# PengjieRen/CaSE_RG

Hardware: AMD Instinct MI355X
Metric: train tokens/sec (query+passage) CaSE model (higher is better)
Workload: dtype bf16; 1 GPU; CaSE train step fwd+bwd+allreduce+clip+Adam+EMA, d_model=512, 6 encoder layers, 10 passages x 384 tok, query 64, answer 40, vocab 30522, per-GPU batch 32, dropout on; global_batch=32, parallelism=dp1

## Files before the change

case_rg_amd/csrc/elementwise.hip:

```cpp
#include "common.h"

namespace {

constexpr int EW_THREADS = 256;

template <typename T>
__global__ void add_kernel(const T* __restrict__ a, const T* __restrict__ b, T* __restrict__ o, int64_t n) {
  for (int64_t i = (int64_t)blockIdx.x * blockDim.x + threadIdx.x; i < n; i += (int64_t)gridDim.x * blockDim.x)
    Elem<T>::st(o + i, Elem<T>::ld(a + i) + Elem<T>::ld(b + i));
}

template <typename T>
__global__ void dropout_kernel(const T* __restrict__ x, T* __restrict__ y, int64_t n, float p, uint64_t seed,
                               uint64_t offset, const CaseStepState* state) {
  offset += rng_base_of(state);
  const float scale = 1.f / (1.f - p);
  for (int64_t i = (int64_t)blockIdx.x * blockDim.x + threadIdx.x; i < n; i += (int64_t)gridDim.x * blockDim.x)
    Elem<T>::st(y + i, rng_uniform(seed, offset + (uint64_t)i) >= p ? Elem<T>::ld(x + i) * scale : 0.f);
}

template <typename T>
__global__ void mask_rows_kernel(const T* __restrict__ x, const uint8_t* __restrict__ valid, T* __restrict__ y,
                                 int64_t rows, int64_t cols) {
  const int64_t n = rows * cols;
// ... 52 lines not shown
      for (int r = 0; r < 8; ++r) t += part[r][c];
      atomicAdd(out + gc, t);
    }
  }
}

template <typename T>
__global__ void add_vec_kernel(const T* __restrict__ a, const T* __restrict__ b, T* __restrict__ o, int64_t nvec) {
  constexpr int E = Vec16<T>::N;
  for (int64_t i = (int64_t)blockIdx.x * blockDim.x + threadIdx.x; i < nvec; i += (int64_t)gridDim.x * blockDim.x) {
    float x[E], y[E];
    Vec16<T>::load(a + i * E, x);
    Vec16<T>::load(b + i * E, y);
#pragma unroll
    for (int e = 0; e < E; ++e) x[e] += y[e];
    Vec16<T>::store(o + i * E, x);
  }
}

struct AddNArgs {
  const void* src[8];
  int n;
};
template <typename T>
__global__ void add_n_vec_kernel(const AddNArgs a, T* __restrict__ o, int64_t nvec) {
  constexpr int E = Vec16<T>::N;
  for (int64_t i = (int64_t)blockIdx.x * blockDim.x + threadIdx.x; i < nvec; i += (int64_t)gridDim.x * blockDim.x) {
    float acc[E], y[E];
    Vec16<T>::load(reinterpret_cast<const T*>(a.src[0]) + i * E, acc);
#pragma unroll
    for (int j = 1; j < 8; ++j) {
      if (j < a.n) {
        Vec16<T>::load(reinterpret_cast<const T*>(a.src[j]) + i * E, y);
#pragma unroll
        for (int e = 0; e < E; ++e) acc[e] += y[e];
      }
    }
    Vec16<T>::store(o + i * E, acc);
  }
}

template <typename T>
__global__ void dropout_vec_kernel(const T* __restrict__ x, T* __restrict__ y, int64_t nvec, float p, uint64_t seed,
                                   uint64_t offset, const CaseStepState* state) {
  offset += rng_base_of(state);
  constexpr int E = Vec16<T>::N;
  const float scale = 1.f / (1.f - p);
  for (int64_t i = (int64_t)blockIdx.x * blockDim.x + threadIdx.x; i < nvec; i += (int64_t)gridDim.x * blockDim.x) {
    float v[E];
    Vec16<T>::load(x + i * E, v);
    const uint64_t idx0 = offset + (uint64_t)(i * E);
    if ((idx0 & 1) == 0) {
#pragma unroll
      for (int e = 0; e < E; e += 2) {
        float u0, u1;
        rng_uniform2(seed, idx0 + e, u0, u1);
        v[e] = u0 >= p ? v[e] * scale : 0.f;
        v[e + 1] = u1 >= p ? v[e + 1] * scale : 0.f;
      }
    } else {
#pragma unroll
      for (int e = 0; e < E; ++e) v[e] = rng_uniform(seed, idx0 + e) >= p ? v[e] * scale : 0.f;
    }
    Vec16<T>::store(y + i * E, v);
  }
}

template <typename T>
__global__ void mask_rows_vec_kernel(const T* __restrict__ x, const uint8_t* __restrict__ valid, T* __restrict__ y,
                                     int64_t rows, int64_t cols) {
  constexpr int E = Vec16<T>::N;
  const int64_t vpr = cols / E, nvec = rows * vpr;
  const bool in_place = x == y;
  for (int64_t i = (int64_t)blockIdx.x * blockDim.x + threadIdx.x; i < nvec; i += (int64_t)gridDim.x * blockDim.x) {
    const bool ok = valid[i / vpr] != 0;
    if (in_place && ok) continue;
    float v[E];
    if (ok) Vec16<T>::load(x + i * E, v);
    else {
#pragma unroll
      for (int e = 0; e < E; ++e) v[e] = 0.f;
    }
    Vec16<T>::store(y + i * E, v);
  }
}

template <typename T>
__global__ __launch_bounds__(256) void rowdot_fwd_kernel(const T* __restrict__ x, const float* __restrict__ w,
                                                         const float* __restrict__ b, float* __restrict__ y, int64_t rows,
                                                         int64_t cols) {
  const int lane = threadIdx.x & 63;
  const int64_t wave = (int64_t)blockIdx.x * 4 + (threadIdx.x >> 6), nwaves = (int64_t)gridDim.x * 4;
  for (int64_t r = wave; r < rows; r += nwaves) {
    float acc = 0.f;
    for (int64_t c = lane; c < cols; c += 64) acc += Elem<T>::ld(x + r * cols + c) * w[c];
    acc = wave_sum(acc);
    if (lane == 0) y[r] = acc + (b ? b[0] : 0.f);
  }
}

struct SkinnyArgs {
  const void* x[4];
  int64_t width[4];
  const float* w; const float* b; float* y;
  int64_t rows, cols;
  int nseg, nout;
};
template <typename T, bool VEC>
__global__ __launch_bounds__(256) void linear_skinny_kernel(const SkinnyArgs a) {
  const int lane = threadIdx.x & 63;
  const int64_t wave = (int64_t)blockIdx.x * 4 + (threadIdx.x >> 6), nwaves = (int64_t)gridDim.x * 4;
  constexpr int NV = Vec16<T>::N;
  for (int64_t r = wave; r < a.rows; r += nwaves) {
    float acc[8] = {0.f, 0.f, 0.f, 0.f, 0.f, 0.f, 0.f, 0.f};
    int64_t off = 0;
#pragma unroll
    for (int k = 0; k < 4; ++k) {
      if (k < a.nseg) {
        const T* xr = reinterpret_cast<const T*>(a.x[k]) + r * a.width[k];
        if constexpr (VEC) {
#pragma unroll 2
          for (int64_t c = (int64_t)lane * NV; c < a.width[k]; c += 64 * NV) {
            float xv[NV];
            Vec16<T>::load(xr + c, xv);
#pragma unroll
            for (int o = 0; o < 8; ++o) {
              if (o < a.nout) {
                const float* wr = a.w + o * a.cols + off + c;
#pragma unroll
                for (int q = 0; q < NV / 4; ++q) {
                  const float4 wv = *reinterpret_cast<const float4*>(wr + 4 * q);
                  acc[o] = fmaf(xv[4 * q], wv.x, acc[o]);
                  acc[o] = fmaf(xv[4 * q + 1], wv.y, acc[o]);
                  acc[o] = fmaf(xv[4 * q + 2], wv.z, acc[o]);
                  acc[o] = fmaf(xv[4 * q + 3], wv.w, acc[o]);
                }
              }
            }
          }
        } else {
          for (int64_t c = lane; c < a.width[k]; c += 64) {
            const float xv = Elem<T>::ld(xr + c);
#pragma unroll
            for (int o = 0; o < 8; ++o)
              if (o < a.nout) acc[o] = fmaf(xv, a.w[o * a.cols + off + c], acc[o]);
          }
        }
        off += a.width[k];
      }
    }
#pragma unroll
    for (int o = 0; o < 8; ++o) {
      if (o < a.nout) {
        const float t = wave_sum(acc[o]);
        if (lane == 0) a.y[r * a.nout + o] = t + (a.b ? a.b[o] : 0.f);
      }
    }
  }
}

template <typename T>
__global__ __launch_bounds__(256) void rowdot_bwd_kernel(const float* __restrict__ g, const T* __restrict__ x,
                                                         const float* __restrict__ w, T* __restrict__ dx,
                                                         float* __restrict__ dw, float* __restrict__ db, int64_t rows,
                                                         int64_t cols, int row_splits) {
  __shared__ float part[4][64];
// ... 343 lines not shown
    }
    Vec16<T>::store(de + r * H + c, ge);
    Vec16<T>::store(da1 + r * H + c, g1);
    Vec16<T>::store(da2 + r * H + c, g2);
  }
}

template <typename T>
__global__ void max_over_p_fwd_kernel(const T* __restrict__ x, T* __restrict__ out, int32_t* __restrict__ arg, int64_t B,
                                      int64_t P, int64_t inner) {
  const int64_t n = B * inner;
  for (int64_t i = (int64_t)blockIdx.x * blockDim.x + threadIdx.x; i < n; i += (int64_t)gridDim.x * blockDim.x) {
    const int64_t b = i / inner, k = i % inner;
    float best = Elem<T>::ld(x + (b * P) * inner + k);
    int32_t bi = 0;
    for (int64_t p = 1; p < P; ++p) {
      const float v = Elem<T>::ld(x + (b * P + p) * inner + k);
      if (v > best) {
        best = v;
        bi = (int32_t)p;
      }
    }
    Elem<T>::st(out + i, best);
    arg[i] = bi;
  }
}

template <typename T>
__global__ void max_over_p_bwd_kernel(const T* __restrict__ d_out, const int32_t* __restrict__ arg, T* __restrict__ dx,
                                      int64_t B, int64_t P, int64_t inner) {
  const int64_t n = B * P * inner;
  for (int64_t i = (int64_t)blockIdx.x * blockDim.x + threadIdx.x; i < n; i += (int64_t)gridDim.x * blockDim.x) {
    const int64_t k = i % inner, bp = i / inner, b = bp / P, p = bp % P;
    Elem<T>::st(dx + i, arg[b * inner + k] == (int32_t)p ? Elem<T>::ld(d_out + b * inner + k) : 0.f);
  }
}

}

#define EW_DISPATCH(what, n_elems, KERNEL, ...)                                                              \
  do {                                                                                                       \
    const int grid = grid_for((n_elems), EW_THREADS, 4);                                                     \
    hipStream_t s_ = (hipStream_t)stream;                                                                    \
    if (dtype == CASE_F32) { typedef float T; hipLaunchKernelGGL(KERNEL<T>, dim3(grid), dim3(EW_THREADS), 0, s_, __VA_ARGS__); } \
    else if (dtype == CASE_BF16) { typedef bf16_t T; hipLaunchKernelGGL(KERNEL<T>, dim3(grid), dim3(EW_THREADS), 0, s_, __VA_ARGS__); } \
    else return case_set_error(CASE_E_UNSUPPORTED, what ": dtype %d", dtype);                              \
    return case_check_launch(what);                                                                          \
  } while (0)

extern "C" int case_add(const void* a, const void* b, void* out, int64_t n, int32_t dtype, case_stream_t stream) {
  CASE_REQUIRE(a && b && out && n > 0, "case_add: bad argument");
  const int ev = dtype == CASE_BF16 ? 8 : 4;
  if (n % ev == 0 && al16(a) && al16(b) && al16(out))
    EW_DISPATCH("case_add", n / ev, add_vec_kernel, (const T*)a, (const T*)b, (T*)out, n / ev);
  EW_DISPATCH("case_add", n, add_kernel, (const T*)a, (const T*)b, (T*)out, n);
}

extern "C" int case_add_n(const void* const* srcs, int32_t count, void* out, int64_t n, int32_t dtype, case_stream_t stream) {
  CASE_REQUIRE(srcs && out && n > 0 && count >= 2 && count <= 8, "case_add_n: bad argument (2 <= count <= 8)");
  const int ev = dtype == CASE_BF16 ? 8 : 4;
  CASE_REQUIRE(n % ev == 0 && al16(out), "case_add_n: element count must be a multiple of %d and the tensors 16-byte aligned", ev);
  AddNArgs a = {};
  a.n = count;
  for (int j = 0; j < count; ++j) {
    CASE_REQUIRE(srcs[j] && al16(srcs[j]), "case_add_n: null or misaligned source %d", j);
    a.src[j] = srcs[j];
  }
  EW_DISPATCH("case_add_n", n / ev, add_n_vec_kernel, a, (T*)out, n / ev);
}

extern "C" int case_dropout(const void* x, void* y, int64_t n, float p, uint64_t seed, uint64_t offset, const CaseStepState* state,
                            int32_t dtype, case_stream_t stream) {
  CASE_REQUIRE(x && y && n > 0 && p >= 0.f && p < 1.f, "case_dropout: bad argument");
  const int ev = dtype == CASE_BF16 ? 8 : 4;
  if (n % ev == 0 && al16(x) && al16(y))
    EW_DISPATCH("case_dropout", n / ev, dropout_vec_kernel, (const T*)x, (T*)y, n / ev, p, seed, offset, state);
  EW_DISPATCH("case_dropout", n, dropout_kernel, (const T*)x, (T*)y, n, p, seed, offset, state);
}

extern "C" int case_mask_rows(const void* x, const uint8_t* row_valid, void* y, int64_t rows, int64_t cols,
                              int32_t dtype, case_stream_t stream) {
  CASE_REQUIRE(x && row_valid && y && rows > 0 && cols > 0, "case_mask_rows: bad argument");
  const int ev = dtype == CASE_BF16 ? 8 : 4;
  if (cols % ev == 0 && al16(x) && al16(y))
    EW_DISPATCH("case_mask_rows", rows * cols / ev, mask_rows_vec_kernel, (const T*)x, row_valid, (T*)y, rows, cols);
  EW_DISPATCH("case_mask_rows", rows * cols, mask_rows_kernel, (const T*)x, row_valid, (T*)y, rows, cols);
}

static int colsum_splits(int64_t rows, int64_t cols) {
  const int64_t col_blocks = (cols + 63) / 64;
  int64_t want = 2048 / col_blocks;
  const int64_t cap = (rows + 31) / 32;
  if (want > cap) want = cap;
  return (int)(want < 1 ? 1 : want);
}

extern "C" int case_colsum(const void* x, float* out, int64_t rows, int64_t cols, int32_t dtype, case_stream_t stream) {
  CASE_REQUIRE(x && out && rows > 0 && cols > 0, "case_colsum: bad argument");
  {
    const int ev = dtype == CASE_BF16 ? 8 : 4;
    if (cols % ev == 0 && al16(x)) {
      const int64_t col_blocks = (cols + 32 * ev - 1) / (32 * ev);
      int64_t want = 2048 / col_blocks, cap = (rows + 63) / 64;
      if (want > cap) want = cap;
      if (want < 1) want = 1;
      const int vsplits = (int)want;
      hipStream_t vs = (hipStream_t)stream;
      if (dtype == CASE_F32) hipLaunchKernelGGL(colsum_vec_kernel<float>, dim3((unsigned)(col_blocks * vsplits)), dim3(256), 0, vs, (const float*)x, out, rows, cols, vsplits);
      else hipLaunchKernelGGL(colsum_vec_kernel<bf16_t>, dim3((unsigned)(col_blocks * vsplits)), dim3(256), 0, vs, (const bf16_t*)x, out, rows, cols, vsplits);
      return case_check_launch("case_colsum");
    }
  }
  const int splits = colsum_splits(rows, cols);
  const int grid = (int)((cols + 63) / 64) * splits;
  hipStream_t s = (hipStream_t)stream;
  if (dtype == CASE_F32) hipLaunchKernelGGL(colsum_kernel<float>, dim3(grid), dim3(256), 0, s, (const float*)x, out, rows, cols, splits);
  else hipLaunchKernelGGL(colsum_kernel<bf16_t>, dim3(grid), dim3(256), 0, s, (const bf16_t*)x, out, rows, cols, splits);
  return case_check_launch("case_colsum");
}

extern "C" int case_cast(const void* x, void* y, int64_t n, int32_t src, int32_t dst, case_stream_t stream) {
  CASE_REQUIRE(x && y && n > 0, "case_cast: bad argument");
  const int grid = grid_for(n, EW_THREADS, 4);
  hipStream_t s = (hipStream_t)stream;
  if (src == CASE_F32 && dst == CASE_BF16) hipLaunchKernelGGL((cast_kernel<float, bf16_t>), dim3(grid), dim3(EW_THREADS), 0, s, (const float*)x, (bf16_t*)y, n);
  else if (src == CASE_BF16 && dst == CASE_F32) hipLaunchKernelGGL((cast_kernel<bf16_t, float>), dim3(grid), dim3(EW_THREADS), 0, s, (const bf16_t*)x, (float*)y, n);
  else if (src == CASE_F32 && dst == CASE_F32) hipLaunchKernelGGL((cast_kernel<float, float>), dim3(grid), dim3(EW_THREADS), 0, s, (const float*)x, (float*)y, n);
  else if (src == CASE_BF16 && dst == CASE_BF16) hipLaunchKernelGGL((cast_kernel<bf16_t, bf16_t>), dim3(grid), dim3(EW_THREADS), 0, s, (const bf16_t*)x, (bf16_t*)y, n);
  else return case_set_error(CASE_E_UNSUPPORTED, "case_cast: dtype");
  return case_check_launch("case_cast");
}

extern "C" int case_scale_cols(const void* x, const float* w, void* y, int64_t rows, int64_t cols, int32_t dtype,
                               case_stream_t stream) {
  CASE_REQUIRE(x && w && y && rows > 0 && cols > 0, "case_scale_cols: bad argument");
  EW_DISPATCH("case_scale_cols", rows * cols, scale_cols_kernel, (const T*)x, w, (T*)y, rows, cols);
}

extern "C" int case_scale_cols_bwd(const void* dy, const void* x, const float* w, void* dx, float* dw, int64_t rows,
                                   int64_t cols, int32_t dtype, case_stream_t stream) {
  CASE_REQUIRE(dy && x && w && dx && dw && rows > 0 && cols > 0, "case_scale_cols_bwd: bad argument");
  const int splits = colsum_splits(rows, cols);
  const int grid = (int)((cols + 63) / 64) * splits;
  hipStream_t s = (hipStream_t)stream;
  if (dtype == CASE_F32) hipLaunchKernelGGL(scale_cols_bwd_kernel<float>, dim3(grid), dim3(256), 0, s, (const float*)dy, (const float*)x, w, (float*)dx, dw, rows, cols, splits);
  else hipLaunchKernelGGL(scale_cols_bwd_kernel<bf16_t>, dim3(grid), dim3(256), 0, s, (const bf16_t*)dy, (const bf16_t*)x, w, (bf16_t*)dx, dw, rows, cols, splits);
  return case_check_launch("case_scale_cols_bwd");
}

extern "C" int case_scale_add_rows(const void* x, const float* pe, void* y, int64_t rows, int64_t seq_len, int64_t H,
                                   float scale, int32_t dtype, case_stream_t stream) {
  CASE_REQUIRE(x && y && rows > 0 && seq_len > 0 && H > 0, "case_scale_add_rows: bad argument");
  EW_DISPATCH("case_scale_add_rows", rows * H, scale_add_rows_kernel, (const T*)x, pe, (T*)y, rows, seq_len, H, scale);
}

extern "C" int case_embed_pos_fwd(const int64_t* ids, const float* table, const float* pe, void* out, int64_t rows,
                                  int64_t seq_len, int64_t H, int64_t vocab, float scale, float drop_p, uint64_t seed,
                                  uint64_t offset, const CaseStepState* state, int32_t dtype, case_stream_t stream) {
  CASE_REQUIRE(ids && table && pe && out && rows > 0 && seq_len > 0 && H > 0 && vocab > 0, "case_embed_pos_fwd: bad argument");
  if ((dtype == CASE_BF16 || dtype == CASE_F32) && H % 8 == 0 && al16(table) && al16(pe) && al16(out) && rows * (H / 8) < (1ll << 31) &&
      seq_len < (1ll << 31)) {
    const unsigned chunks = (unsigned)(rows * (H / 8));
    const dim3 grid((unsigned)grid_for(chunks, 256, 1, 256 * 16));
    hipStream_t s_ = (hipStream_t)stream;
    if (dtype == CASE_F32)
      hipLaunchKernelGGL(embed_pos_fwd_vec_kernel<float>, grid, dim3(256), 0, s_, ids, table, pe, (float*)out, chunks, (unsigned)seq_len,
// ... 146 lines not shown
```

case_rg_amd/csrc/rowops.hip:

```cpp
#include <stdlib.h>

#ifndef CASE_STREAM_DEFAULT_POLICY
#define CASE_VEC16_NT
#endif
#include "common.h"

namespace {

constexpr int LN_THREADS = 256;
constexpr int LN_MAXPT = 16;

template <typename T>
__global__ __launch_bounds__(LN_THREADS) void ln_fwd_kernel(const T* __restrict__ x, const T* __restrict__ x2,
                                                            const float* __restrict__ gamma,
                                                            const float* __restrict__ beta, T* __restrict__ y,
                                                            float* __restrict__ mean, float* __restrict__ rstd,
                                                            int64_t rows, int64_t cols, float eps) {
  __shared__ float red[32];
  for (int64_t r = blockIdx.x; r < rows; r += gridDim.x) {
    const T* xr = x + r * cols;
    const T* x2r = x2 ? x2 + r * cols : nullptr;
    float s = 0.f;
    for (int64_t c = threadIdx.x; c < cols; c += LN_THREADS) s += Elem<T>::ld(xr + c) + (x2r ? Elem<T>::ld(x2r + c) : 0.f);
    const float mu = block_sum(s, red) / (float)cols;
// ... 48 lines not shown
    const float m1 = block_sum(s1, red) / (float)cols;
    const float m2 = block_sum(s2, red) / (float)cols;
    T* dxr = dx + r * cols;
#pragma unroll
    for (int i = 0; i < LN_MAXPT; ++i) {
      const int64_t c = threadIdx.x + (int64_t)i * LN_THREADS;
      if (c < cols) {
        const float xh = (Elem<T>::ld(xr + c) + (x2r ? Elem<T>::ld(x2r + c) : 0.f) - mu) * rs;
        const float g = Elem<T>::ld(dyr + c) * gamma[c];
        Elem<T>::st(dxr + c, rs * (g - m1 - xh * m2) + (dx_add ? Elem<T>::ld(dx_add + r * cols + c) : 0.f));
      }
    }
  }
#pragma unroll
  for (int i = 0; i < LN_MAXPT; ++i) {
    const int64_t c = threadIdx.x + (int64_t)i * LN_THREADS;
    if (c < cols) {
      atomicAdd(d_gamma + c, acc_g[i]);
      atomicAdd(d_beta + c, acc_b[i]);
    }
  }
}

constexpr int LNV_MAX = 8;

template <typename T, int NV>
__global__ __launch_bounds__(256) void ln_fwd_vec_kernel(const T* __restrict__ x, const T* __restrict__ x2,
                                                         const float* __restrict__ gamma, const float* __restrict__ beta,
                                                         T* __restrict__ y, float* __restrict__ mean,
                                                         float* __restrict__ rstd, int64_t rows, int64_t cols, float eps) {
  constexpr int E = Vec16<T>::N;
  const int lane = threadIdx.x & 63;
  const int64_t wave = (int64_t)blockIdx.x * 4 + (threadIdx.x >> 6), nwaves = (int64_t)gridDim.x * 4;
  for (int64_t r = wave; r < rows; r += nwaves) {
    float v[NV][E];
    float s = 0.f;
#pragma unroll
    for (int i = 0; i < NV; ++i) {
      const int64_t c = ((int64_t)i * 64 + lane) * E;
      if (c < cols) {
        Vec16<T>::load(x + r * cols + c, v[i]);
        if (x2) {
          float w[E];
          Vec16<T>::load(x2 + r * cols + c, w);
#pragma unroll
          for (int e = 0; e < E; ++e) v[i][e] += w[e];
        }
#pragma unroll
        for (int e = 0; e < E; ++e) s += v[i][e];
      }
    }
    const float mu = wave_sum(s) / (float)cols;
    float q = 0.f;
#pragma unroll
    for (int i = 0; i < NV; ++i)
      if (((int64_t)i * 64 + lane) * E < cols) {
#pragma unroll
        for (int e = 0; e < E; ++e) q += (v[i][e] - mu) * (v[i][e] - mu);
      }
    const float rs = rsqrtf(wave_sum(q) / (float)cols + eps);
    if (lane == 0) {
      mean[r] = mu;
      rstd[r] = rs;
    }
#pragma unroll
    for (int i = 0; i < NV; ++i) {
      const int64_t c = ((int64_t)i * 64 + lane) * E;
      if (c < cols) {
        float g[E], b[E], o[E];
#pragma unroll
        for (int e = 0; e < E; e += 4) {
          const float4 gg = *reinterpret_cast<const float4*>(gamma + c + e), bb = *reinterpret_cast<const float4*>(beta + c + e);
          g[e] = gg.x; g[e + 1] = gg.y; g[e + 2] = gg.z; g[e + 3] = gg.w;
          b[e] = bb.x; b[e + 1] = bb.y; b[e + 2] = bb.z; b[e + 3] = bb.w;
        }
#pragma unroll
        for (int e = 0; e < E; ++e) o[e] = (v[i][e] - mu) * rs * g[e] + b[e];
        Vec16<T>::store(y + r * cols + c, o);
      }
    }
  }
}

template <typename T, int NV>
__global__ __launch_bounds__(256) void ln_bwd_vec_guarded_kernel(const T* __restrict__ dy, const T* __restrict__ x,
                                                         const T* __restrict__ x2, const float* __restrict__ gamma,
                                                         const float* __restrict__ mean, const float* __restrict__ rstd,
                                                         T* __restrict__ dx, const T* __restrict__ dx_add,
                                                         float* __restrict__ d_gamma, float* __restrict__ d_beta, int64_t rows,
                                                         int64_t cols) {
  constexpr int E = Vec16<T>::N;
  extern __shared__ float part[];
  const int lane = threadIdx.x & 63, wid = threadIdx.x >> 6;
  const int64_t wave = (int64_t)blockIdx.x * 4 + wid, nwaves = (int64_t)gridDim.x * 4;
  float ag[NV][E], ab[NV][E], g[NV][E];
#pragma unroll
  for (int i = 0; i < NV; ++i) {
    const int64_t c = ((int64_t)i * 64 + lane) * E;
#pragma unroll
    for (int e = 0; e < E; ++e) {
      ag[i][e] = ab[i][e] = 0.f;
      g[i][e] = c < cols ? gamma[c + e] : 0.f;
    }
  }
  for (int64_t r = wave; r < rows; r += nwaves) {
    const float mu = mean[r], rs = rstd[r];
    float xh[NV][E], gy[NV][E];
    float s1 = 0.f, s2 = 0.f;
#pragma unroll
    for (int i = 0; i < NV; ++i) {
      const int64_t c = ((int64_t)i * 64 + lane) * E;
      if (c < cols) {
        float d[E];
        Vec16<T>::load(x + r * cols + c, xh[i]);
        if (x2) {
          float w[E];
          Vec16<T>::load(x2 + r * cols + c, w);
#pragma unroll
          for (int e = 0; e < E; ++e) xh[i][e] += w[e];
        }
        Vec16<T>::load(dy + r * cols + c, d);
#pragma unroll
        for (int e = 0; e < E; ++e) {
          xh[i][e] = (xh[i][e] - mu) * rs;
          gy[i][e] = d[e] * g[i][e];
          s1 += gy[i][e];
          s2 += gy[i][e] * xh[i][e];
          ag[i][e] += d[e] * xh[i][e];
          ab[i][e] += d[e];
        }
      }
    }
    const float m1 = wave_sum(s1) / (float)cols, m2 = wave_sum(s2) / (float)cols;
#pragma unroll
    for (int i = 0; i < NV; ++i) {
      const int64_t c = ((int64_t)i * 64 + lane) * E;
      if (c < cols) {
        float o[E];
#pragma unroll
        for (int e = 0; e < E; ++e) o[e] = rs * (gy[i][e] - m1 - xh[i][e] * m2);
        if (dx_add) {
          float w[E];
          Vec16<T>::load(dx_add + r * cols + c, w);
#pragma unroll
          for (int e = 0; e < E; ++e) o[e] += w[e];
        }
        Vec16<T>::store(dx + r * cols + c, o);
      }
    }
  }
  for (int w = 1; w < 4; ++w) {
    if (wid == w) {
#pragma unroll
      for (int i = 0; i < NV; ++i) {
        const int64_t c = ((int64_t)i * 64 + lane) * E;
        if (c < cols) {
#pragma unroll
          for (int e = 0; e < E; ++e) {
            part[c + e] = ag[i][e];
            part[cols + c + e] = ab[i][e];
          }
        }
      }
    }
    __syncthreads();
    if (wid == 0) {
// ... 30 lines not shown
  void* out;
  float p;
  uint64_t seed, offset;
  const CaseStepState* state;
};
template <typename T, typename V = Vec16<T>>
__device__ __forceinline__ void ln_store_dropped(const LnDrop& dr, int64_t idx, const float (&o)[V::N]) {
  constexpr int E = V::N;
  float q[E];
  if constexpr (sizeof(T) == 2) {
#pragma unroll
    for (int i = 0; i < E; i += 2) {
      const uint32_t w = f32x2_to_bf16x2(o[i], o[i + 1]);
      q[i] = __uint_as_float(w << 16);
      q[i + 1] = __uint_as_float(w & 0xffff0000u);
    }
  } else {
#pragma unroll
    for (int e = 0; e < E; ++e) q[e] = o[e];
  }
  const float scale = 1.f / (1.f - dr.p);
#pragma unroll
  for (int e = 0; e < E; e += 2) {
    float u0, u1;
    rng_uniform2(dr.seed, dr.offset + rng_base_of(dr.state) + (uint64_t)(idx + e), u0, u1);
    q[e] = u0 >= dr.p ? q[e] * scale : 0.f;
    q[e + 1] = u1 >= dr.p ? q[e + 1] * scale : 0.f;
  }
  V::store(reinterpret_cast<T*>(dr.out) + idx, q);
}

template <typename T, int NV, bool HAS_X2, bool HAS_ADD, bool DROP2 = false, typename V = Vec16<T>>
__global__ __launch_bounds__(256) void ln_bwd_vec_kernel(const T* __restrict__ dy, const T* __restrict__ x,
                                                         const T* __restrict__ x2, const float* __restrict__ gamma,
                                                         const float* __restrict__ mean, const float* __restrict__ rstd,
                                                         T* __restrict__ dx, const T* __restrict__ dx_add,
                                                         float* __restrict__ d_gamma, float* __restrict__ d_beta, int64_t rows,
                                                         int64_t cols, const LnDrop dr = LnDrop()) {
  constexpr int E = V::N;
  typedef typename V::raw raw_t;
  extern __shared__ float part[];
  const int lane = threadIdx.x & 63, wid = threadIdx.x >> 6;
  const int64_t wave = (int64_t)blockIdx.x * 4 + wid, nwaves = (int64_t)gridDim.x * 4;
  float ag[NV][E], ab[NV][E], g[NV][E];
#pragma unroll
  for (int i = 0; i < NV; ++i) {
    const int64_t c = ((int64_t)i * 64 + lane) * E;
#pragma unroll
    for (int e = 0; e < E; ++e) {
      ag[i][e] = ab[i][e] = 0.f;
      g[i][e] = gamma[c + e];
    }
  }
  struct Raw {
    raw_t x[NV], d[NV], x2[HAS_X2 ? NV : 1], add[HAS_ADD ? NV : 1];
    float mu, rs;
  };
  auto request = [&](Raw& w, int64_t r) {
    const int64_t base = r * cols + (int64_t)lane * E;
    w.mu = mean[r];
    w.rs = rstd[r];
#pragma unroll
    for (int i = 0; i < NV; ++i) {
      const int64_t o = base + (int64_t)i * 64 * E;
      w.x[i] = *reinterpret_cast<const raw_t*>(x + o);
      w.d[i] = *reinterpret_cast<const raw_t*>(dy + o);
      if constexpr (HAS_X2) w.x2[i] = *reinterpret_cast<const raw_t*>(x2 + o);
      if constexpr (HAS_ADD) w.add[i] = *reinterpret_cast<const raw_t*>(dx_add + o);
    }
  };
  auto normalised = [&](const Raw& w, int i, float (&xh)[E]) {
    V::unpack(w.x[i], xh);
    if constexpr (HAS_X2) {
      float t[E];
      V::unpack(w.x2[i], t);
#pragma unroll
      for (int e = 0; e < E; ++e) xh[e] += t[e];
    }
#pragma unroll
    for (int e = 0; e < E; ++e) xh[e] = (xh[e] - w.mu) * w.rs;
  };
  Raw cur, nxt;
  request(cur, wave < rows ? wave : rows - 1);
  for (int64_t r = wave; r < rows; r += nwaves) {
    request(nxt, r + nwaves < rows ? r + nwaves : rows - 1);
    float s1 = 0.f, s2 = 0.f;
#pragma unroll
    for (int i = 0; i < NV; ++i) {
      float xh[E], d[E];
      normalised(cur, i, xh);
      V::unpack(cur.d[i], d);
#pragma unroll
      for (int e = 0; e < E; ++e) {
        const float gy = d[e] * g[i][e];
        s1 += gy;
        s2 = fmaf(gy, xh[e], s2);
        ag[i][e] = fmaf(d[e], xh[e], ag[i][e]);
        ab[i][e] += d[e];
      }
    }
    const float m1 = wave_sum(s1) / (float)cols, m2 = wave_sum(s2) / (float)cols;
#pragma unroll
    for (int i = 0; i < NV; ++i) {
      float xh[E], d[E], o[E];
      normalised(cur, i, xh);
      V::unpack(cur.d[i], d);
#pragma unroll
      for (int e = 0; e < E; ++e) o[e] = cur.rs * fmaf(-xh[e], m2, fmaf(d[e], g[i][e], -m1));
      if constexpr (HAS_ADD) {
        float w[E];
        V::unpack(cur.add[i], w);
#pragma unroll
        for (int e = 0; e < E; ++e) o[e] += w[e];
      }
      V::store(dx + r * cols + ((int64_t)i * 64 + lane) * E, o);
      if constexpr (DROP2) ln_store_dropped<T, V>(dr, r * cols + ((int64_t)i * 64 + lane) * E, o);
    }
    cur = nxt;
  }
  float* mine = part + (int64_t)wid * 2 * cols;
#pragma unroll
  for (int i = 0; i < NV; ++i) {
    const int64_t c = ((int64_t)i * 64 + lane) * E;
#pragma unroll
    for (int e = 0; e < E; ++e) {
      mine[c + e] = ag[i][e];
      mine[cols + c + e] = ab[i][e];
    }
  }
  __syncthreads();
  for (int64_t c = threadIdx.x; c < 2 * cols; c += 256) {
    const float t = part[c] + part[2 * cols + c] + part[4 * cols + c] + part[6 * cols + c];
    atomicAdd(c < cols ? d_gamma + c : d_beta + (c - cols), t);
  }
}

template <typename T, int R, bool HAS_X2, bool HAS_ADD, bool DROP2 = false, typename V = Vec16<T>, int MAXW = 8>
__global__ __launch_bounds__(64 * MAXW) void ln_bwd_split_kernel(const T* __restrict__ dy, const T* __restrict__ x,
                                                           const T* __restrict__ x2, const float* __restrict__ gamma,
                                                           const float* __restrict__ mean, const float* __restrict__ rstd,
                                                           T* __restrict__ dx, const T* __restrict__ dx_add,
                                                           float* __restrict__ d_gamma, float* __restrict__ d_beta, int64_t rows,
                                                           int64_t cols, const LnDrop dr = LnDrop()) {
  constexpr int E = V::N;
  typedef typename V::raw raw_t;
  __shared__ float part[2][R][MAXW][2];
  const int lane = threadIdx.x & 63, wid = threadIdx.x >> 6, nw = blockDim.x >> 6;
  const int64_t col = ((int64_t)wid * 64 + lane) * E;
  float ag[E], ab[E], g[E];
#pragma unroll
  for (int e = 0; e < E; ++e) {
    ag[e] = ab[e] = 0.f;
    g[e] = gamma[col + e];
  }
  struct Raw {
    raw_t x[R], d[R], x2[HAS_X2 ? R : 1], add[HAS_ADD ? R : 1];
    float mu[R], rs[R];
  };
  auto request = [&](Raw& w, int64_t row0) {
#pragma unroll
    for (int j = 0; j < R; ++j) {
      const int64_t r = row0 + j < rows ? row0 + j : rows - 1;
      const int64_t o = r * cols + col;
      w.mu[j] = mean[r];
      w.rs[j] = rstd[r];
      w.x[j] = *reinterpret_cast<const raw_t*>(x + o);
// ... 9 lines not shown
      V::unpack(w.x2[j], t);
#pragma unroll
      for (int e = 0; e < E; ++e) xh[e] += t[e];
    }
#pragma unroll
    for (int e = 0; e < E; ++e) xh[e] = (xh[e] - w.mu[j]) * w.rs[j];
  };
  const int64_t stride = (int64_t)gridDim.x * R;
  Raw cur, nxt;
  int buf = 0;
  if ((int64_t)blockIdx.x * R < rows) request(cur, (int64_t)blockIdx.x * R);
  for (int64_t row0 = (int64_t)blockIdx.x * R; row0 < rows; row0 += stride, buf ^= 1) {
#pragma unroll
    for (int j = 0; j < R; ++j) {
      float xh[E], d[E];
      normalised(cur, j, xh);
      V::unpack(cur.d[j], d);
      float s1 = 0.f, s2 = 0.f;
      const bool real = row0 + j < rows;
#pragma unroll
      for (int e = 0; e < E; ++e) {
        const float gy = d[e] * g[e];
        s1 += gy;
        s2 = fmaf(gy, xh[e], s2);
        if (real) {
          ag[e] = fmaf(d[e], xh[e], ag[e]);
          ab[e] += d[e];
        }
      }
      s1 = wave_sum(s1);
      s2 = wave_sum(s2);
      if (lane == 0) {
        part[buf][j][wid][0] = s1;
        part[buf][j][wid][1] = s2;
      }
    }
    if (row0 + stride < rows) request(nxt, row0 + stride);
    __syncthreads();
#pragma unroll
    for (int j = 0; j < R; ++j) {
      float m1 = 0.f, m2 = 0.f;
      for (int w = 0; w < nw; ++w) {
        m1 += part[buf][j][w][0];
        m2 += part[buf][j][w][1];
      }
      m1 /= (float)cols;
      m2 /= (float)cols;
      if (row0 + j < rows) {
        float xh[E], d[E], o[E];
        normalised(cur, j, xh);
        V::unpack(cur.d[j], d);
#pragma unroll
        for (int e = 0; e < E; ++e) o[e] = cur.rs[j] * fmaf(-xh[e], m2, fmaf(d[e], g[e], -m1));
        if constexpr (HAS_ADD) {
          float w[E];
          V::unpack(cur.add[j], w);
#pragma unroll
          for (int e = 0; e < E; ++e) o[e] += w[e];
        }
        V::store(dx + (row0 + j) * cols + col, o);
        if constexpr (DROP2) ln_store_dropped<T, V>(dr, (row0 + j) * cols + col, o);
      }
    }
    cur = nxt;
  }
  extern __shared__ float cpart[];
  __syncthreads();
#pragma unroll
  for (int e = 0; e < E; ++e) {
    cpart[col + e] = ag[e];
    cpart[cols + col + e] = ab[e];
  }
  __syncthreads();
  for (int64_t c = threadIdx.x; c < 2 * cols; c += blockDim.x) atomicAdd(c < cols ? d_gamma + c : d_beta + (c - cols), cpart[c]);
}

template <typename T>
bool ln_vec_ok(const void* a, const void* b, const void* c, int64_t cols) {
  constexpr int E = Vec16<T>::N;
  auto al = [](const void* p) { return p == nullptr || ((uintptr_t)p % 16 == 0); };
  return cols % E == 0 && cols <= (int64_t)LNV_MAX * 64 * E && al(a) && al(b) && al(c);
}

template <typename T>
void ln_fwd_vec_launch(const void* x, const void* x2, const float* gamma, const float* beta, void* y, float* mean,
                       float* rstd, int64_t rows, int64_t cols, float eps, hipStream_t s) {
  constexpr int E = Vec16<T>::N;
  const int nv = (int)((cols + 64 * E - 1) / (64 * E));
  const int grid = grid_for(rows, 4, 1, 256 * 16);
#define LNF(NVV) hipLaunchKernelGGL((ln_fwd_vec_kernel<T, NVV>), dim3(grid), dim3(256), 0, s, (const T*)x, (const T*)x2, gamma, beta, (T*)y, mean, rstd, rows, cols, eps)
  switch (nv) { case 1: LNF(1); break; case 2: LNF(2); break; case 3: LNF(3); break; case 4: LNF(4); break;
                case 5: LNF(5); break; case 6: LNF(6); break; case 7: LNF(7); break; default: LNF(8); break; }
#undef LNF
}

template <typename T>
void ln_bwd_vec_launch(const void* dy, const void* x, const void* x2, const float* gamma, const float* mean,
                       const float* rstd, void* dx, const void* dx_add, float* dg, float* db, int64_t rows, int64_t cols,
                       hipStream_t s) {
  constexpr int E = Vec16<T>::N;
  const int nv = (int)((cols + 64 * E - 1) / (64 * E));
  if constexpr (sizeof(T) == 2) {
    if (cols % 256 == 0 && cols % 512 != 0 && cols <= 1280) {
      const int grid = grid_for(rows, 4, 8, 256 * 8);
      const size_t lds = 8 * cols * sizeof(float);
#define LN8(NVV, X2, ADD) hipLaunchKernelGGL((ln_bwd_vec_kernel<T, NVV, X2, ADD, false, Vec8<T>>), dim3(grid), dim3(256), lds, s, (const T*)dy, (const T*)x, (const T*)x2, gamma, mean, rstd, (T*)dx, (const T*)dx_add, dg, db, rows, cols)
#define LN8B(NVV) do { if (x2 && dx_add) LN8(NVV, true, true); else if (x2) LN8(NVV, true, false); else if (dx_add) LN8(NVV, false, true); else LN8(NVV, false, false); } while (0)
      if (cols == 256) LN8B(1);
      else if (cols == 768) LN8B(3);
      else LN8B(5);
#undef LN8B
#undef LN8
      return;
    }
    if (cols % 256 == 0 && cols % 512 != 0 && cols <= 15 * 256) {
      constexpr int R = 2;
      const int nw = (int)(cols / 256);
      const int grid = grid_for(rows, 1, R * 16, 256 * 4);
#define LNS8(X2, ADD) hipLaunchKernelGGL((ln_bwd_split_kernel<T, R, X2, ADD, false, Vec8<T>, 16>), dim3(grid), dim3(64 * nw), 2 * cols * sizeof(float), s, (const T*)dy, (const T*)x, (const T*)x2, gamma, mean, rstd, (T*)dx, (const T*)dx_add, dg, db, rows, cols)
      if (x2 && dx_add) LNS8(true, true);
      else if (x2) LNS8(true, false);
      else if (dx_add) LNS8(false, true);
      else LNS8(false, false);
#undef LNS8
      return;
    }
  }
  if (cols != (int64_t)nv * 64 * E || nv > 8) {
    const int grid = grid_for(rows, 4, 16, 256 * 4);
    const size_t lds = 2 * cols * sizeof(float);
#define LNG(NVV) hipLaunchKernelGGL((ln_bwd_vec_guarded_kernel<T, NVV>), dim3(grid), dim3(256), lds, s, (const T*)dy, (const T*)x, (const T*)x2, gamma, mean, rstd, (T*)dx, (const T*)dx_add, dg, db, rows, cols)
    switch (nv) { case 1: LNG(1); break; case 2: LNG(2); break; case 3: LNG(3); break; case 4: LNG(4); break;
                  case 5: LNG(5); break; case 6: LNG(6); break; case 7: LNG(7); break; default: LNG(8); break; }
#undef LNG
    return;
  }
  if (nv >= 3) {
    constexpr int R = 2;
    const int grid = grid_for(rows, 1, R * 16, 256 * 4);
#define LNS(X2, ADD) hipLaunchKernelGGL((ln_bwd_split_kernel<T, R, X2, ADD>), dim3(grid), dim3(64 * nv), 2 * cols * sizeof(float), s, (const T*)dy, (const T*)x, (const T*)x2, gamma, mean, rstd, (T*)dx, (const T*)dx_add, dg, db, rows, cols)
    if (x2 && dx_add) LNS(true, true);
    else if (x2) LNS(true, false);
    else if (dx_add) LNS(false, true);
    else LNS(false, false);
#undef LNS
    return;
  }
  const int grid = grid_for(rows, 4, 8, 256 * 8);
  const size_t lds = 8 * cols * sizeof(float);
#define LNB(NVV, X2, ADD) hipLaunchKernelGGL((ln_bwd_vec_kernel<T, NVV, X2, ADD>), dim3(grid), dim3(256), lds, s, (const T*)dy, (const T*)x, (const T*)x2, gamma, mean, rstd, (T*)dx, (const T*)dx_add, dg, db, rows, cols)
#define LNB2(NVV) do { if (x2 && dx_add) LNB(NVV, true, true); else if (x2) LNB(NVV, true, false); else if (dx_add) LNB(NVV, false, true); else LNB(NVV, false, false); } while (0)
  if (nv == 1) LNB2(1);
  else LNB2(2);
#undef LNB2
#undef LNB
}

template <int TPR>
__device__ __forceinline__ float row_max(float v, float* red) {
  if constexpr (TPR == 64) return wave_max(v);
  else return block_max(v, red);
}
template <int TPR>
__device__ __forceinline__ float row_sum(float v, float* red) {
  if constexpr (TPR == 64) return wave_sum(v);
  else return block_sum(v, red);
}

template <typename TI, typename TO, int TPR>
__global__ __launch_bounds__(256) void softmax_fwd_kernel(const CaseSoftmaxDesc d, const TI* __restrict__ x,
                                                          const uint8_t* __restrict__ col_valid,
// ... 538 lines not shown
```

Measured before the change: 1.317 million tokens/s.

## Add streaming row-masking and prefetching LayerNorm forward kernels

Adds a wave-per-row-group mask_rows kernel that handles several rows per wave, skips loads for invalid rows and reads a zero vector instead of branching. It also adds a LayerNorm forward kernel that double-buffers the next row's loads (optionally nontemporal) while computing the current row, with gamma/beta held in registers or LDS and half-wave handling for widths like 768. An explicit waitcnt is inserted before the LN backward loop. The new paths are on by default behind an env switch; they aim to cut memory latency stalls in these bandwidth-bound row ops, at the cost of more register pressure and hand-scheduled code.

```diff
diff --git a/case_rg_amd/csrc/elementwise.hip b/case_rg_amd/csrc/elementwise.hip
--- a/case_rg_amd/csrc/elementwise.hip
+++ b/case_rg_amd/csrc/elementwise.hip
@@ -158,6 +158,50 @@
       for (int e = 0; e < E; ++e) v[e] = 0.f;
     }
     Vec16<T>::store(y + i * E, v);
+  }
+}
+
+constexpr int MASK_G = 4, MASK_MAX_GRID = 256 * 8;
+__device__ const uint4 mask_zero_vec = {0u, 0u, 0u, 0u};
+
+template <bool IN_PLACE>
+__global__ __launch_bounds__(256) void mask_rows_stream_kernel(const char* __restrict__ x, const uint8_t* __restrict__ valid, char* __restrict__ y,
+                                                               int64_t rows, int vpr) {
+  typedef unsigned int u32x4 __attribute__((ext_vector_type(4)));
+  typedef const __attribute__((address_space(1))) u32x4* gvec_t;
+  const gvec_t zero = (gvec_t)(uintptr_t)&mask_zero_vec;
+  const int lane = threadIdx.x & 63;
+  const int64_t wave = (int64_t)blockIdx.x * 4 + __builtin_amdgcn_readfirstlane(threadIdx.x >> 6), nwaves = (int64_t)gridDim.x * 4;
+  const int64_t row_bytes = (int64_t)vpr * 16;
+  for (int64_t r0 = wave * MASK_G; r0 < rows; r0 += nwaves * MASK_G) {
+    if (r0 + MASK_G <= rows) {
+      bool ok[MASK_G];
+#pragma unroll
+      for (int g = 0; g < MASK_G; ++g) ok[g] = valid[r0 + g] != 0;
+      for (int j = lane; j < vpr; j += 64) {
+        const int64_t at = r0 * row_bytes + (int64_t)j * 16;
+        if constexpr (IN_PLACE) {
+#pragma unroll
+          for (int g = 0; g < MASK_G; ++g)
+            if (!ok[g]) *reinterpret_cast<u32x4*>(y + at + g * row_bytes) = u32x4{0u, 0u, 0u, 0u};
+        } else {
+          u32x4 v[MASK_G];
+#pragma unroll
+          for (int g = 0; g < MASK_G; ++g) v[g] = *(ok[g] ? (gvec_t)(uintptr_t)(x + at + g * row_bytes) : zero);
+#pragma unroll
+          for (int g = 0; g < MASK_G; ++g) *reinterpret_cast<u32x4*>(y + at + g * row_bytes) = v[g];
+        }
+      }
+    } else {
+      for (int64_t r = r0; r < rows; ++r) {
+        const bool ok = valid[r] != 0;
+        if (IN_PLACE && ok) continue;
+        for (int j = lane; j < vpr; j += 64) {
+          const int64_t at = r * row_bytes + (int64_t)j * 16;
+          *reinterpret_cast<u32x4*>(y + at) = *(!IN_PLACE && ok ? (gvec_t)(uintptr_t)(x + at) : zero);
+        }
+      }
+    }
   }
 }
 
@@ -667,6 +711,14 @@
                               int32_t dtype, case_stream_t stream) {
   CASE_REQUIRE(x && row_valid && y && rows > 0 && cols > 0, "case_mask_rows: bad argument");
   const int ev = dtype == CASE_BF16 ? 8 : 4;
+  const char* sw = getenv("CASE_ROW_STREAM");
+  if (!(sw && sw[0] == '0') && (dtype == CASE_F32 || dtype == CASE_BF16) && cols % ev == 0 && cols / ev <= INT32_MAX && al16(x) && al16(y)) {
+    const int grid = grid_for(rows, 4, MASK_G, MASK_MAX_GRID), vpr = (int)(cols / ev);
+    hipStream_t s_ = (hipStream_t)stream;
+    if (x == y) hipLaunchKernelGGL(mask_rows_stream_kernel<true>, dim3(grid), dim3(256), 0, s_, (const char*)x, row_valid, (char*)y, rows, vpr);
+    else hipLaunchKernelGGL(mask_rows_stream_kernel<false>, dim3(grid), dim3(256), 0, s_, (const char*)x, row_valid, (char*)y, rows, vpr);
+    return case_check_launch("case_mask_rows");
+  }
   if (cols % ev == 0 && al16(x) && al16(y))
     EW_DISPATCH("case_mask_rows", rows * cols / ev, mask_rows_vec_kernel, (const T*)x, row_valid, (T*)y, rows, cols);
   EW_DISPATCH("case_mask_rows", rows * cols, mask_rows_kernel, (const T*)x, row_valid, (T*)y, rows, cols);
diff --git a/case_rg_amd/csrc/rowops.hip b/case_rg_amd/csrc/rowops.hip
--- a/case_rg_amd/csrc/rowops.hip
+++ b/case_rg_amd/csrc/rowops.hip
@@ -154,6 +154,122 @@
   }
 }
 
+template <typename T>
+__device__ __forceinline__ uint4 ln_load_raw(const T* p) {
+#ifdef CASE_VEC16_NT
+  typedef unsigned int u32x4_nt __attribute__((ext_vector_type(4)));
+  const u32x4_nt t = __builtin_nontemporal_load(reinterpret_cast<const u32x4_nt*>(p));
+  return make_uint4(t[0], t[1], t[2], t[3]);
+#else
+  return *reinterpret_cast<const uint4*>(p);
+#endif
+}
+
+template <typename T, int NV, bool HAS_X2, bool HALF>
+__global__ __launch_bounds__(256) void ln_fwd_stream_kernel(const T* __restrict__ x, const T* __restrict__ x2,
+                                                            const float* __restrict__ gamma, const float* __restrict__ beta,
+                                                            T* __restrict__ y, float* __restrict__ mean, float* __restrict__ rstd,
+                                                            int64_t rows, int64_t cols, float eps) {
+#pragma clang fp contract(off)
+  constexpr int E = Vec16<T>::N;
+  constexpr bool GB_LDS = NV * E > 16;
+  extern __shared__ float gb[];
+  const int lane = threadIdx.x & 63;
+  const int64_t wave = (int64_t)blockIdx.x * 4 + (threadIdx.x >> 6), nwaves = (int64_t)gridDim.x * 4;
+  const bool tail_on = !HALF || lane < 32;
+  auto col = [&](int i) { return (i * 64 + (HALF && i == NV - 1 ? (lane & 31) : lane)) * E; };
+  float g[GB_LDS ? 1 : NV][E], b[GB_LDS ? 1 : NV][E];
+  auto params = [&](int i, float (&gi)[E], float (&bi)[E], const float* gsrc, const float* bsrc) {
+#pragma unroll
+    for (int e = 0; e < E; e += 4) {
+      const float4 gg = *reinterpret_cast<const float4*>(gsrc + col(i) + e), bb = *reinterpret_cast<const float4*>(bsrc + col(i) + e);
+      gi[e] = gg.x; gi[e + 1] = gg.y; gi[e + 2] = gg.z; gi[e + 3] = gg.w;
+      bi[e] = bb.x; bi[e + 1] = bb.y; bi[e + 2] = bb.z; bi[e + 3] = bb.w;
+    }
+  };
+  if constexpr (GB_LDS) {
+    for (int c = threadIdx.x; c < (int)cols; c += 256) {
+      gb[c] = gamma[c];
+      gb[cols + c] = beta[c];
+    }
+    __syncthreads();
+  } else {
+#pragma unroll
+    for (int i = 0; i < NV; ++i) params(i, g[i], b[i], gamma, beta);
+  }
+  struct Raw {
+    uint4 x[NV], x2[HAS_X2 ? NV : 1];
+  };
+  auto request = [&](Raw& w, int64_t r) {
+#pragma unroll
+    for (int i = 0; i < NV; ++i) {
+      w.x[i] = ln_load_raw(x + r * cols + col(i));
+      if constexpr (HAS_X2) w.x2[i] = ln_load_raw(x2 + r * cols + col(i));
+    }
+  };
+  auto value = [&](const Raw& w, int i, float (&v)[E]) {
+    Vec16<T>::unpack(w.x[i], v);
+    if constexpr (HAS_X2) {
+      float t[E];
+      Vec16<T>::unpack(w.x2[i], t);
+#pragma unroll
+      for (int e = 0; e < E; ++e) v[e] += t[e];
+    }
+  };
+  Raw cur, nxt;
+  request(cur, wave < rows ? wave : rows - 1);
+  __builtin_amdgcn_sched_barrier(0);
+  __builtin_amdgcn_s_waitcnt(0x0F70);
+  __builtin_amdgcn_sched_barrier(0);
+  for (int64_t r = wave; r < rows; r += nwaves) {
+    request(nxt, r + nwaves < rows ? r + nwaves : rows - 1);
+    __builtin_amdgcn_sched_barrier(0);
+    int fresh = 0;
+    asm volatile("" : "+v"(fresh));
+    float s = 0.f;
+#pragma unroll
+    for (int i = 0; i < NV; ++i) {
+      float v[E];
+      value(cur, i, v);
+#pragma unroll
+      for (int e = 0; e < E; ++e) s += (HALF && i == NV - 1 && !tail_on) ? 0.f : v[e];
+    }
+    const float mu = wave_sum(s) / (float)cols;
+    float q = 0.f;
+#pragma unroll
+    for (int i = 0; i < NV; ++i) {
+      float v[E];
+      value(cur, i, v);
+#pragma unroll
+      for (int e = 0; e < E; ++e) {
+        const float d = v[e] - mu;
+        q += (HALF && i == NV - 1 && !tail_on) ? 0.f : d * d;
+      }
+    }
+    const float rs = rsqrtf(wave_sum(q) / (float)cols + eps);
+    if (lane == 0) {
+      mean[r] = mu;
+      rstd[r] = rs;
+    }
+#pragma unroll
+    for (int i = 0; i < NV; ++i) {
+      float v[E], o[E];
+      value(cur, i, v);
+      if constexpr (GB_LDS) {
+        float gi[E], bi[E];
+        params(i, gi, bi, gb + fresh, gb + cols + fresh);
+#pragma unroll
+        for (int e = 0; e < E; ++e) o[e] = fmaf((v[e] - mu) * rs, gi[e], bi[e]);
+      } else {
+#pragma unroll
+        for (int e = 0; e < E; ++e) o[e] = fmaf((v[e] - mu) * rs, g[i][e], b[i][e]);
+      }
+      if (!(HALF && i == NV - 1) || tail_on) Vec16<T>::store(y + r * cols + col(i), o);
+    }
+    cur = nxt;
+  }
+}
+
 template <typename T, int NV>
 __global__ __launch_bounds__(256) void ln_bwd_vec_guarded_kernel(const T* __restrict__ dy, const T* __restrict__ x,
                                                          const T* __restrict__ x2, const float* __restrict__ gamma,
@@ -350,6 +466,9 @@
   };
   Raw cur, nxt;
   request(cur, wave < rows ? wave : rows - 1);
+  __builtin_amdgcn_sched_barrier(0);
+  __builtin_amdgcn_s_waitcnt(0x0F70);
+  __builtin_amdgcn_sched_barrier(0);
   for (int64_t r = wave; r < rows; r += nwaves) {
     request(nxt, r + nwaves < rows ? r + nwaves : rows - 1);
     float s1 = 0.f, s2 = 0.f;
@@ -525,11 +644,35 @@
   return cols % E == 0 && cols <= (int64_t)LNV_MAX * 64 * E && al(a) && al(b) && al(c);
 }
 
+constexpr int LN_FWD_ROWS_PER_WAVE = 4, LN_FWD_MAX_GRID = 256 * 8;
+
 template <typename T>
 void ln_fwd_vec_launch(const void* x, const void* x2, const float* gamma, const float* beta, void* y, float* mean,
                        float* rstd, int64_t rows, int64_t cols, float eps, hipStream_t s) {
   constexpr int E = Vec16<T>::N;
   const int nv = (int)((cols + 64 * E - 1) / (64 * E));
+  const char* sw = getenv("CASE_ROW_STREAM");
+  if (!(sw && sw[0] == '0')) {
+    const bool whole = cols == (int64_t)nv * 64 * E;
+    const bool half = sizeof(T) == 2 && cols % 512 == 256 && nv <= 3;
+    if ((whole || half) && nv >= 2) {
+      const int sgrid = grid_for(rows, 4, LN_FWD_ROWS_PER_WAVE, LN_FWD_MAX_GRID);
+      const size_t lds = nv * E > 16 ? 2 * cols * sizeof(float) : 0;
+#define LNS(NVV, X2, HALF) hipLaunchKernelGGL((ln_fwd_stream_kernel<T, NVV, X2, HALF>), dim3(sgrid), dim3(256), lds, s, (const T*)x, (const T*)x2, gamma, beta, (T*)y, mean, rstd, rows, cols, eps)
+#define LNS2(NVV, HALF) do { if (x2) LNS(NVV, true, HALF); else LNS(NVV, false, HALF); } while (0)
+      if constexpr (sizeof(T) == 2) {
+        if (half) {
+          if (nv == 2) LNS2(2, true); else LNS2(3, true);
+          return;
+        }
+      }
+      switch (nv) { case 2: LNS2(2, false); break; case 3: LNS2(3, false); break; case 4: LNS2(4, false); break;
+                    case 5: LNS2(5, false); break; case 6: LNS2(6, false); break; case 7: LNS2(7, false); break; default: LNS2(8, false); break; }
+#undef LNS2
+#undef LNS
+      return;
+    }
+  }
   const int grid = grid_for(rows, 4, 1, 256 * 16);
 #define LNF(NVV) hipLaunchKernelGGL((ln_fwd_vec_kernel<T, NVV>), dim3(grid), dim3(256), 0, s, (const T*)x, (const T*)x2, gamma, beta, (T*)y, mean, rstd, rows, cols, eps)
   switch (nv) { case 1: LNF(1); break; case 2: LNF(2); break; case 3: LNF(3); break; case 4: LNF(4); break;
```

Measured after the change: 1.310 million tokens/s (median of 3 runs). About the same (-0.5%).
